# tier4/lidar_feature_extraction

Measured on AMD Instinct MI355X. Metric: scans/sec (64-ring x 1800 synthetic scans, extraction hot path, inputs resident in HBM), higher is better.
Workload: dtype f64

## Files before the change

### lidar_feature_extraction_amd/csrc/lfx_api.hip

```cpp
#include "lfx_internal.hpp"

#include <algorithm>
#include <cstddef>
#include "lfx_kernels_extract.hpp"

#ifdef LFX_TEST_HOOKS
#define LFX_DEBUG_ENV(name) std::getenv("LFX_DEBUG_" name)
#else
#define LFX_DEBUG_ENV(name) static_cast<const char *>(nullptr)
#endif

using namespace lfx_host;

namespace
{

std::string g_create_error;

const char * kKernelNames[LFX_N_KERNELS] = {
  "ring_scatter_kernel", "ring_unit_kernel", "ring_order_kernel", "ring_unit_kernel(second pass)", "ring_extract_kernel",
  "ring_totals_kernel", "feature_compact_kernel", "ring_unit_org_kernel", "ring_cut_kernel", "fallback_tail_kernel", "grid_count_kernel",
  "batch_reset_kernel", "ring_long_kernel",
  "pose_graph_linearize_kernel", "pose_graph_node_kernel", "pose_graph_reduce_kernel", "pose_graph_chain_factor_kernel",
  "pose_graph_chain_solve_kernel", "pose_graph_s_assemble_kernel", "pose_graph_s_diag_kernel", "pose_graph_s_panel_kernel",
  "pose_graph_s_update_kernel", "pose_graph_s_solve_kernel", "pose_graph_step_kernel"};

int64_t ordered_key(double d)
{
  int64_t k;
  std::memcpy(&k, &d, 8);
  return k < 0 ? std::numeric_limits<int64_t>::min() - k : k;
}

double from_ordered_key(int64_t k)
{
  const int64_t b = k < 0 ? std::numeric_limits<int64_t>::min() - k : k;
  double d;
  std::memcpy(&d, &b, 8);
  return d;
}

double cos_bound(double radian_threshold)
{
  if (!(std::acos(1.0) < radian_threshold)) {return std::numeric_limits<double>::infinity();}
  if (std::acos(-1.0) < radian_threshold) {return -1.0;}
  int64_t lo = ordered_key(-1.0), hi = ordered_key(1.0);
  while (hi - lo > 1) {
    const int64_t mid = lo + (hi - lo) / 2;
    if (std::acos(from_ordered_key(mid)) < radian_threshold) {hi = mid;} else {lo = mid;}
  }
  return from_ordered_key(hi);
}

}

std::string & lfx_host::create_error() {return g_create_error;}

namespace
{

struct Timed : TimedSpan
{
  Timed(lfx_ctx * c, KernelSlot k, hipStream_t s)
  : TimedSpan(c, c->profile_now, k, s) {}
};

int drain_spans(lfx_ctx * c)
{
  for (auto & sp : c->spans) {
    LFX_HIP(c, hipEventSynchronize(sp.b));
    float t = 0.f;
    LFX_HIP(c, hipEventElapsedTime(&t, sp.a, sp.b));
    c->ms[sp.k] += t;
    c->launches[sp.k] += 1;
    c->free_events.push_back(sp.a);
    c->free_events.push_back(sp.b);
  }
  c->spans.clear();
  return LFX_OK;
}

int validate_params(const lfx_params * p, std::string & why)
{
  if (!p) {why = "params is NULL"; return LFX_ERR_INVALID_ARGUMENT;}
  if (p->padding <= 0 || p->padding > LFX_MAX_PADDING) {
    why = "convolution_padding must be in [1, " + std::to_string(LFX_MAX_PADDING) + "]";
    return LFX_ERR_INVALID_ARGUMENT;
  }
  if (p->n_blocks <= 0) {why = "n_blocks must be > 0"; return LFX_ERR_INVALID_ARGUMENT;}
  if (!(p->neighbor_degree_threshold > 0) || !(p->distance_diff_threshold > 0) ||
    !(p->parallel_beam_min_range_ratio > 0) || !(p->edge_threshold > 0) || !(p->surface_threshold > 0) ||
    !(p->min_range > 0) || !(p->max_range > 0))
  {
    why = "every threshold / range parameter must be > 0 (hyper_parameter.hpp:45-53)";
    return LFX_ERR_INVALID_ARGUMENT;
  }
  return LFX_OK;
}

lfx::Params device_params(const lfx_params & p)
{
  lfx::Params d;
  d.P = p.padding;
  d.B = p.n_blocks;
  d.cos_bound = cos_bound(p.neighbor_degree_threshold * M_PI / 180.0);
  d.cos_bound_f = (float)d.cos_bound;
  d.dist_diff = p.distance_diff_threshold;
  d.pb_ratio = p.parallel_beam_min_range_ratio;
  d.pb_ratio_f = (float)d.pb_ratio;
  d.edge_thr = p.edge_threshold;
  d.surf_thr = p.surface_threshold;
  d.min_range = p.min_range;
  d.max_range = p.max_range;
  return d;
}

int debug_pin(const char * value) {return value ? (std::atoi(value) != 0 ? 1 : 0) : -1;}

// ... 131 lines not shown
      const uint32_t R = c->max_rings;
      const int P = c->dev.P, B = c->dev.B;
      for (uint32_t s = 0; s < batch; s++) {
        const uint32_t n = n_points[s], C = n / R;
        if (C * R != n || C == 0u || C > c->cap) {continue;}
        uint32_t * g = c->h_scan_geom.data() + (size_t)s * lfx::kGeomStride;
        g[0] = C;
        for (int j = 0; j <= B && j <= lfx::kUnitMaxBlocks; j++) {g[1 + j] = (uint32_t)lfx::block_boundary((int)C, P, B, j);}
      }
      LFX_HIP(c, hipMemcpyAsync(c->scan_geom.p, c->h_scan_geom.data(), c->h_scan_geom.size() * 4, hipMemcpyHostToDevice, st));
    }
  }
  c->last_batch = batch;
  c->last_points = d_points;
  c->deskewed_in_place = false;
  c->profile_now = c->profiling && (c->batch_no++ % c->profile_every) == 0u;
  const uint32_t par = c->parity;
  const AccSet acc = acc_set(c, par), other = acc_set(c, par ^ 1u);
  uint32_t * const counters = acc.counters;
  const lfx::UnitTables * unit_tab = c->unit_tab.p + par;
  uint32_t * defer_count = counters + lfx::kCntDefer, * redo_count = counters + lfx::kCntRedo,
    * slow_count = counters + lfx::kCntSlow, * fb_count = counters + lfx::kCntFallback;
  const uint8_t * pts = static_cast<const uint8_t *>(d_points);
  const uint32_t chunks = (longest + lfx::kChunkPoints - 1) / lfx::kChunkPoints;
  const bool canon = canonical_layout(c->layout) && (reinterpret_cast<uintptr_t>(pts) & 15u) == 0;
  if (c->long_slices != 0u) {
    LFX_HIP(c, hipMemsetAsync(c->long_count.p, 0, 4, st));
  }
  if (c->h_counters) {
    const uint32_t end = __atomic_load_n(c->h_counters + 1 + lfx::kCounters, __ATOMIC_ACQUIRE);
    uint32_t got[lfx::kCounters];
    for (int i = 0; i < lfx::kCounters; i++) {got[i] = __atomic_load_n(c->h_counters + 1 + i, __ATOMIC_RELAXED);}
    __atomic_thread_fence(__ATOMIC_ACQUIRE);
    const uint32_t begin = __atomic_load_n(c->h_counters, __ATOMIC_RELAXED);
    if (end != 0u && end == begin && end != c->report_taken) {
      static_assert(sizeof(c->route.report) == sizeof(got), "the report is the counters block");
      std::memcpy(c->route.report, got, sizeof(got));
      c->route.report_rings = got[lfx::kCntBatch] * c->max_rings;
      c->report_taken = end;
    }
  }
  const RouteChoice choice = choose_route(c->route, c->route_pins, c->fused_possible && canon && chunks != 0, batch, c->max_rings);
  const bool fused = choice.fused, short_tail = choice.short_tail;
  const bool holes = choice.holes && c->drop_zero != 0u && c->cum16.p != nullptr;
  const uint32_t fb_grid = choice.fb_grid;
  if (chunks == 0) {
    LFX_HIP(c, hipMemsetAsync(c->scan_info.p, 0, (size_t)batch * 16, st));
    LFX_HIP(c, hipMemsetAsync(c->ring_count.p, 0, (size_t)batch * lfx::kRings * 4, st));
    return LFX_OK;
  }
  const bool lazy = fused && short_tail && !choice.xform;
  if (!lazy || c->aux_dirty != 0u) {
    const uint32_t n_aux = c->aux_dirty > batch ? c->aux_dirty : batch;
    Timed t(c, kSlotReset, st);
    hipLaunchKernelGGL(lfx::batch_reset_kernel, dim3(64), dim3(256), 0, st,
      c->chunk_flags.p, n_aux * c->max_chunks, c->ring_flags.p, n_aux * (uint32_t)lfx::kRings, counters, c->fb_list.p, batch,
      fused ? 0u : 1u, c->xform.p);
    c->aux_dirty = lazy ? 0u : batch;
  }
  c->last_used_xform = fused && choice.xform;
  if (fused) {
    const bool xf = choice.xform;
    if (xf) {
      Timed t(c, kSlotCut, st);
      hipLaunchKernelGGL(lfx::ring_cut_kernel, dim3(batch), dim3(lfx::kCutThreads), 0, st,
        pts, c->scan_begin.p, c->max_rings, c->cap, c->xform.p, counters);
    }
    const uint32_t groups = (c->max_rings + 3u) / 4u;
    if (holes) {
      Timed t(c, kSlotGridCount, st);
      const uint32_t row_words = c->cap / lfx::kPieceCols + 1u;
      const size_t count_lds = ((size_t)c->max_rings * row_words + 2u * groups * (size_t)c->dev.B) * 4u;
      auto count_pass = [&](auto kernel, dim3 grid, uint32_t threads, size_t lds, auto... more) {
          hipLaunchKernelGGL(kernel, grid, dim3(threads), lds, st,
            pts, c->scan_begin.p, c->scan_geom.p, c->max_rings, lfx::cum_stride(c->cap), c->cum16.p, c->ring_count.p, unit_tab, counters,
            c->hole_desc.p, c->cap, 64u * c->unit_chunks, 4u * (uint32_t)lfx::holes_loads((int)c->unit_chunks), more...);
        };
      if (batch >= c->scan_count_from && count_lds <= 144u * 1024u) {
        count_pass(lfx::scan_count_kernel, dim3(batch), lfx::kScanCountThreads, count_lds, row_words);
      } else {
        count_pass(lfx::grid_count_kernel, dim3(groups, batch), 256u, 0);
      }
    }
    {
      Timed t(c, kSlotUnitOrg, st);
      const UnitOrgArgs a{c->dev, c->cap, c->unit_flags, c->max_rings, c->drop_zero, pts, c->scan_begin.p, c->ring_count.p, unit_tab,
        c->xform.p, c->scan_geom.p};
      launch_unit_org(c->unit_variant, (int)c->unit_chunks, xf, holes, dim3(groups, (uint32_t)c->dev.B, batch), c->unit_lds_pad, st, a);
    }
  }
  const lfx::RingExtractArgs ex{c->dev, c->cap, c->stage_flags, c->max_rings, pts, c->layout, c->scan_begin.p, c->ring_count.p, c->sxy.p, c->sz.p,
    c->sidx.p, c->label_s.p, (c->outputs & LFX_OUT_CURVATURE) ? c->curv_s.p : nullptr, c->rec_pts.p, c->rec_idx.p, c->ring_status.p,
    c->unit_ne.p, c->unit_ns.p, c->unit_span.p, c->ring_flags.p, c->long_count.p, c->long_list.p,
    (uint32_t)(c->long_list.n / 2u)};
  const lfx::ScatterArgs sc{pts, c->layout, c->scan_begin.p, c->chunk_base.p, c->chunk_flags.p, c->ring_count.p, c->scan_info.p, acc.scan_flags,
    c->sxy.p, c->sz.p, c->sidx.p, c->max_chunks, c->max_rings, c->cap, c->drop_zero};
  if (lazy) {
    Timed t(c, kSlotTail, st);
    const uint32_t turns = (batch + lfx::kTailMaxTurns - 1u) / lfx::kTailMaxTurns;
    const uint32_t rows = fb_grid < 2u ? fb_grid : 2u;
    const dim3 grid(chunks, rows > turns ? rows : turns);
    if (canon) {
      hipLaunchKernelGGL(lfx::fallback_tail_kernel<true>, grid, dim3(lfx::kChunkThreads), c->ring_lds, st, sc, ex, fb_count, c->fb_list.p, c->tail_ticket.p);
    } else {
      hipLaunchKernelGGL(lfx::fallback_tail_kernel<false>, grid, dim3(lfx::kChunkThreads), c->ring_lds, st, sc, ex, fb_count, c->fb_list.p, c->tail_ticket.p);
    }
  } else {
    {
      Timed t(c, kSlotScatter, st);
      auto kern = &lfx::ring_scatter_kernel<false>;
      if (canon) {kern = &lfx::ring_scatter_kernel<true>;}
      if (fb_grid == batch) {
        kern = canon ? &lfx::ring_scatter_kernel<true, true> : &lfx::ring_scatter_kernel<false, true>;
      }
      hipLaunchKernelGGL(kern, dim3(chunks, fb_grid), dim3(lfx::kChunkThreads), 0, st,
        sc.pts, sc.L, sc.scan_begin, sc.chunk_base, sc.chunk_flags, sc.ring_count, sc.scan_info, sc.scan_flags,
        sc.sxy, sc.sz, sc.sidx, sc.max_chunks, sc.max_rings, sc.cap, sc.drop_zero, fb_count, c->fb_list.p,
        c->slot_id.empty() ? nullptr : c->ring_slot.p);
    }
    const uint32_t list_grid = fused ? (c->slow_grid < 4u * fb_grid ? c->slow_grid : 4u * fb_grid) : c->slow_grid;
    if (c->fast_path && !short_tail) {
      auto order_pass = [&](uint32_t grid, uint32_t all_rings, uint32_t redo_cap, uint32_t list_cover) {
          Timed t(c, kSlotOrder, st);
          hipLaunchKernelGGL(lfx::ring_order_kernel, dim3(grid), dim3(512), c->order_lds, st,
            c->cap, c->max_rings, c->ring_count.p, c->sxy.p, c->sz.p, c->sidx.p, c->ring_flags.p, defer_count,
            c->defer_list.p, redo_count, c->redo_list.p, slow_count, c->slow_list.p, all_rings, counters + lfx::kCntPreFixed, redo_cap,
            fb_count, c->fb_list.p, list_cover);
        };
      c->pre_order = choice.pre_order;
      if (c->pre_order) {order_pass(fused ? list_grid : 4 * c->slow_grid, 1u, 0u, 0u);}
      {
        Timed t(c, kSlotUnit, st);
        const uint32_t units = c->max_rings * (uint32_t)c->dev.B;
        const UnitArgs a{c->dev, c->cap, c->unit_flags, c->max_rings, c->ring_count.p, c->sxy.p, c->sz.p, c->sidx.p, unit_tab,
          defer_count, c->defer_list.p, fb_count, c->fb_list.p, 0u};
        launch_unit(c->unit_variant, false, (int)c->unit_chunks, fused, dim3((units + lfx::kUnitWaves - 1) / lfx::kUnitWaves, fb_grid),
          c->unit_lds_pad, st, a);
      }
      const uint32_t redo_cap = choice.redo_cap;
      order_pass(list_grid, 0u, redo_cap, 0xFFFFFFFFu );
      {
        Timed t(c, kSlotUnitSecond, st);
        const uint32_t units = redo_cap * (uint32_t)c->dev.B;
        const UnitArgs a{c->dev, c->cap, c->unit_flags, c->max_rings, c->ring_count.p, c->sxy.p, c->sz.p, c->sidx.p, unit_tab,
          slow_count, c->slow_list.p, redo_count, c->redo_list.p, redo_cap};
        launch_unit(c->unit_variant, true, (int)c->unit_chunks, false, dim3((units + lfx::kUnitWaves - 1) / lfx::kUnitWaves), c->unit_lds_pad, st, a);
      }
    }
    {
      Timed t(c, kSlotExtract, st);
      const dim3 grid = c->fast_path ? dim3(list_grid) : dim3(c->max_rings, batch);
      hipLaunchKernelGGL(lfx::ring_extract_kernel, grid, dim3(c->ring_threads), c->ring_lds, st,
        ex, short_tail ? 2u : (c->fast_path ? 1u : 0u), short_tail ? fb_count : slow_count, short_tail ? c->fb_list.p : c->slow_list.p);
    }
  }
  if (c->long_slices != 0u) {
    Timed t(c, kSlotLong, st);
    hipLaunchKernelGGL(lfx::ring_long_kernel, dim3(c->long_slices), dim3(512), lfx::kLongSortLds, st, ex, c->long_work.p,
      c->long_slice_bytes);
  }
  {
    const uint32_t n_units = c->fast_path ? (uint32_t)c->dev.B : 1u;
    const bool self_totals = (fused || (uint64_t)batch * c->max_rings <= 8192u) && c->totals_env != 1;
    if (!self_totals) {
      Timed t(c, kSlotTotals, st);
      hipLaunchKernelGGL(lfx::ring_totals_kernel, dim3(batch), dim3(lfx::kRings), 0, st,
        c->scan_info.p, c->ring_count.p, c->unit_ne.p, c->unit_ns.p, acc.ring_nedge, acc.ring_nsurf,
        c->ring_ebase.p, c->ring_sbase.p, n_units, c->max_rings);
    }
    c->batch_serial = c->batch_serial + 1u == 0u ? 1u : c->batch_serial + 1u;
    {
      Timed t(c, kSlotCompact, st);
      hipLaunchKernelGGL(lfx::feature_compact_kernel, dim3((c->max_rings + 3) / 4, batch), dim3(256), 0, st,
        n_units, c->cap, c->scan_begin.p, c->ring_count.p, self_totals ? nullptr : c->ring_ebase.p, c->ring_sbase.p, c->unit_ne.p,
        c->unit_ns.p, c->unit_span.p, c->rec_pts.p, c->rec_idx.p, c->edge_pts.p, c->edge_idx.p, c->surf_pts.p,
        c->surf_idx.p, c->max_rings, c->scan_info.p, counters, c->h_counters, c->batch_serial, acc.ring_nedge, acc.ring_nsurf, c->rec32.p,
        c->slot_places, acc.scan_flags, c->ring_count.p, batch, fused ? 1u : 0u,
        other.counters, other.scan_flags, other.ring_nedge, other.ring_nsurf, c->par_dirty[par ^ 1u]);
    }
    c->par_dirty[par ^ 1u] = 0u;
    c->par_dirty[par] = batch;
    c->parity = par ^ 1u;
  }
  LFX_HIP(c, hipGetLastError());
  return LFX_OK;
}

size_t align16(size_t v) {return (v + 15u) & ~(size_t)15u;}

struct FetchPlan
{
  uint32_t first = 0, count = 0, p0 = 0, mask = 0;
  size_t o_hdr = 0, o_ep = 0, o_sp = 0, o_cv = 0, o_ei = 0, o_si = 0, o_sx = 0, o_lb = 0;
  uint8_t * H = nullptr;
  std::vector<uint32_t> begin;
};

int fetch_queue(lfx_ctx * c, uint32_t first, uint32_t count, hipStream_t st, uint32_t mask, PinnedBuf & block, FetchPlan & plan)
{
  if (count == 0 || first + count > c->last_batch) {return fail(c, LFX_ERR_INVALID_ARGUMENT, "scan index outside the last batch");}
  const uint32_t p0 = c->h_scan_begin[first];
  const size_t P = c->h_scan_begin[first + count] - p0;
  mask &= c->outputs | ~(uint32_t)LFX_OUT_CURVATURE;
  const bool want_lab = mask & LFX_OUT_LABELS, want_curv = mask & LFX_OUT_CURVATURE, want_sidx = mask & LFX_OUT_SORTED_INDEX;
  const size_t o_hdr = 0, o_ep = align16((size_t)count * lfx::kResultHeaderBytes), o_sp = o_ep + P * 16, o_cv = o_sp + P * 16,
    o_ei = o_cv + (want_curv ? P * 8 : 0), o_si = o_ei + P * 4, o_sx = o_si + P * 4, o_lb = o_sx + (want_sidx ? P * 4 : 0),
    total = o_lb + (want_lab ? P : 0) + 16;
  if (block.reserve(total) != hipSuccess) {return fail(c, LFX_ERR_OUT_OF_MEMORY, "cannot allocate the pinned result block");}
  uint8_t * H = block.p;
  plan.first = first; plan.count = count; plan.p0 = p0; plan.mask = mask; plan.H = H;
  plan.o_hdr = o_hdr; plan.o_ep = o_ep; plan.o_sp = o_sp; plan.o_cv = o_cv; plan.o_ei = o_ei; plan.o_si = o_si; plan.o_sx = o_sx; plan.o_lb = o_lb;
  plan.begin.assign(c->h_scan_begin.begin() + first, c->h_scan_begin.begin() + first + count + 1);
  hipLaunchKernelGGL(lfx::result_pack_kernel, dim3(8, count), dim3(256), 0, st,
    first, p0, c->scan_begin.p, c->scan_info.p, c->ring_count.p, c->ring_status.p, c->edge_pts.p, c->edge_idx.p,
    c->surf_pts.p, c->surf_idx.p, H + o_hdr, reinterpret_cast<float4 *>(H + o_ep), reinterpret_cast<float4 *>(H + o_sp),
    reinterpret_cast<uint32_t *>(H + o_ei), reinterpret_cast<uint32_t *>(H + o_si));
  LFX_HIP(c, hipGetLastError());
  if ((want_lab || want_curv || want_sidx) && P) {
    if (c->d_sidx.n < P) {
      LFX_HIP(c, hipStreamSynchronize(st));
      c->d_label.release(); c->d_curv.release(); c->d_sidx.release();
      if (c->d_label.alloc(P) != hipSuccess || c->d_curv.alloc(P) != hipSuccess || c->d_sidx.alloc(P) != hipSuccess) {
        return fail(c, LFX_ERR_OUT_OF_MEMORY, "cannot allocate the per-point output buffers");
      }
    }
    LFX_HIP(c, hipMemsetAsync(c->d_label.p, 0, P, st));
// ... 895 lines not shown
```

### lidar_feature_extraction_amd/csrc/lfx_internal.hpp

```cpp
#pragma once

#include "../../include/lfx.h"

#include <hip/hip_runtime.h>

#include <cmath>
#include <cstdio>
#include <cstdlib>
#include <cstring>
#include <limits>
#include <string>
#include <type_traits>
#include <utility>
#include <vector>

#include "lfx_kernels_common.hpp"

namespace lfx_host
{

constexpr int kUnitVariantPadding[4] = {5, 5, 2, 0};

struct UnitOrgArgs
{
  lfx::Params prm;
  uint32_t cap, flags, max_rings, drop_zero;
  const uint8_t * pts;
  const uint32_t * scan_begin;
  uint32_t * ring_count;
  const lfx::UnitTables * tab;
  const uint32_t * xform, * geom;
};
struct UnitArgs
{
  lfx::Params prm;
  uint32_t cap, flags, max_rings;
  const uint32_t * ring_count;
  const float2 * sxy;
  const float * sz;
  const uint32_t * sidx;
  const lfx::UnitTables * tab;
  uint32_t * defer_count, * defer_list;
  const uint32_t * list_count, * list;
  uint32_t redo_cap;
};
#define LFX_DECLARE_UNIT_LAUNCHERS(V) \
  void launch_unit_org_v##V(int chunks, bool xf, bool holes, dim3 grid, uint32_t lds_pad, hipStream_t st, const UnitOrgArgs & a); \
  void launch_unit_v##V(bool second, int chunks, bool loop, dim3 grid, uint32_t lds_pad, hipStream_t st, const UnitArgs & a);
LFX_DECLARE_UNIT_LAUNCHERS(0) LFX_DECLARE_UNIT_LAUNCHERS(1) LFX_DECLARE_UNIT_LAUNCHERS(2) LFX_DECLARE_UNIT_LAUNCHERS(3)
#undef LFX_DECLARE_UNIT_LAUNCHERS
inline void launch_unit_org(int variant, int chunks, bool xf, bool holes, dim3 grid, uint32_t lds_pad, hipStream_t st, const UnitOrgArgs & a)
{
  switch (variant) {
    case 0: launch_unit_org_v0(chunks, xf, holes, grid, lds_pad, st, a); break;
    case 1: launch_unit_org_v1(chunks, xf, holes, grid, lds_pad, st, a); break;
    case 2: launch_unit_org_v2(chunks, xf, holes, grid, lds_pad, st, a); break;
    default: launch_unit_org_v3(chunks, xf, holes, grid, lds_pad, st, a); break;
  }
}
inline void launch_unit(int variant, bool second, int chunks, bool loop, dim3 grid, uint32_t lds_pad, hipStream_t st, const UnitArgs & a)
{
  switch (variant) {
    case 0: launch_unit_v0(second, chunks, loop, grid, lds_pad, st, a); break;
    case 1: launch_unit_v1(second, chunks, loop, grid, lds_pad, st, a); break;
    case 2: launch_unit_v2(second, chunks, loop, grid, lds_pad, st, a); break;
    default: launch_unit_v3(second, chunks, loop, grid, lds_pad, st, a); break;
  }
}

template<typename T>
struct DevBuf
{
  T * p = nullptr;
  size_t n = 0;
  DevBuf() = default;
  DevBuf(const DevBuf &) = delete;
  DevBuf & operator=(const DevBuf &) = delete;
  DevBuf(DevBuf && o) noexcept : p(o.p), n(o.n) {o.p = nullptr; o.n = 0;}
  DevBuf & operator=(DevBuf && o) noexcept
  {
    if (this != &o) {release(); p = o.p; n = o.n; o.p = nullptr; o.n = 0;}
    return *this;
  }
  ~DevBuf() {release();}
  hipError_t alloc(size_t count)
  {
    release();
    const hipError_t e = hipMalloc(reinterpret_cast<void **>(&p), count * sizeof(T) + 16);
    if (e == hipSuccess) {n = count;} else {p = nullptr;}
    return e;
  }
  void release()
  {
    if (p) {(void)hipFree(p);}
    p = nullptr;
    n = 0;
  }
};
static_assert(!std::is_copy_constructible_v<DevBuf<float>> && !std::is_copy_assignable_v<DevBuf<float>>, "a device buffer has one owner");

template<typename T>
hipError_t hold(DevBuf<T> & b, size_t need, bool exact = false)
{
  if (b.n >= need && (b.p || need == 0)) {return hipSuccess;}
  return b.alloc(exact ? need : need + need / 2);
}

struct HostScan
{
  std::vector<uint8_t> ring_status;
  std::vector<uint32_t> ring_count, ring_offset;
  std::vector<uint16_t> ring_id;
};

struct PinnedBuf
{
  uint8_t * p = nullptr;
  size_t bytes = 0;
  PinnedBuf() = default;
// ... 212 lines not shown

  bool profiling = false;
  uint32_t profile_every = 1, batch_no = 0;
  bool profile_now = false;
  struct Span { hipEvent_t a, b; int k; };
  std::vector<Span> spans;
  std::vector<hipEvent_t> free_events;
  double ms[LFX_N_KERNELS] = {};
  uint64_t launches[LFX_N_KERNELS] = {};
};

namespace lfx_host
{

std::string & create_error();

inline hipEvent_t take_event(lfx_ctx * c)
{
  if (!c->free_events.empty()) {
    hipEvent_t e = c->free_events.back();
    c->free_events.pop_back();
    return e;
  }
  hipEvent_t e = nullptr;
  (void)hipEventCreate(&e);
  return e;
}
struct TimedSpan
{
  TimedSpan(lfx_ctx * c, bool on, int k, hipStream_t s)
  : c_(c), on_(on), k_(k), s_(s)
  {
    if (on_) {
      a_ = take_event(c_);
      b_ = take_event(c_);
      (void)hipEventRecord(a_, s_);
    }
  }
  ~TimedSpan()
  {
    if (on_) {
      (void)hipEventRecord(b_, s_);
      c_->spans.push_back({a_, b_, k_});
    }
  }
  TimedSpan(const TimedSpan &) = delete;
  TimedSpan & operator=(const TimedSpan &) = delete;
  lfx_ctx * c_;
  bool on_;
  int k_;
  hipStream_t s_;
  hipEvent_t a_ = nullptr, b_ = nullptr;
};

#define LFX_HIP(ctx, call) \
  do { \
    const hipError_t e_ = (call); \
    if (e_ != hipSuccess) { \
      (ctx)->err = std::string(#call) + ": " + hipGetErrorString(e_); \
      return LFX_ERR_HIP; \
    } \
  } while (0)

inline int fail(lfx_ctx * ctx, int code, const std::string & msg)
{
  if (ctx) {ctx->err = msg;}
  return code;
}

inline int Tail::order_behind(lfx_ctx * c, hipStream_t st) const
{
  if (pending) {LFX_HIP(c, hipStreamWaitEvent(st, event, 0));}
  return LFX_OK;
}
inline int Tail::done(lfx_ctx * c, hipStream_t st) const
{
  if (!event) {LFX_HIP(c, hipEventCreateWithFlags(&event, hipEventDisableTiming));}
  LFX_HIP(c, hipEventRecord(event, st));
  pending = true;
  return LFX_OK;
}
inline int Tail::settle(lfx_ctx * c) const
{
  if (pending) {LFX_HIP(c, hipEventSynchronize(event)); pending = false;}
  return LFX_OK;
}

inline int TableSlot::take(lfx_ctx * c, size_t doubles, hipError_t & mem)
{
  const int rs = used.settle(c);
  if (rs != LFX_OK) {return rs;}
  mem = h.reserve(sizeof(double) * doubles);
  if (mem == hipSuccess) {mem = hold(d, doubles);}
  return LFX_OK;
}

inline int check_device(lfx_ctx * c, int device, const char * what)
{
  if (device != c->device) {return fail(c, LFX_ERR_INVALID_ARGUMENT, std::string(what) + " lives on another device");}
  return LFX_OK;
}

inline bool finite_all(const double * v, size_t n)
{
  for (size_t i = 0; i < n; i++) {
    if (!std::isfinite(v[i])) {return false;}
// ... 123 lines not shown
```

### lidar_feature_extraction_amd/csrc/lfx_kernels_extract.hpp

```cpp
#pragma once

#include "lfx_kernels_common.hpp"

#pragma clang fp contract(off)

namespace lfx
{

__global__ __launch_bounds__(256) void batch_reset_kernel(
  uint32_t * __restrict__ chunk_flags, uint32_t n_flags, uint32_t * __restrict__ ring_flags, uint32_t n_rflags,
  uint32_t * __restrict__ counters , uint32_t * __restrict__ fb_list, uint32_t batch,
  uint32_t all_fall_back ,
  uint32_t * __restrict__ xform )
{
  const uint32_t i = blockIdx.x * blockDim.x + threadIdx.x, stride = gridDim.x * blockDim.x;
  for (uint32_t k = i; k < n_flags; k += stride) {chunk_flags[k] = 0;}
  for (uint32_t k = i; k < n_rflags; k += stride) {ring_flags[k] = 0; xform[k] = 0;}
  if (all_fall_back) {
    for (uint32_t k = i; k < batch; k += stride) {fb_list[k] = k;}
    if (i == 0) {counters[kCntFallback] = batch;}
  }
}

constexpr uint32_t kSpinLimit = 200000;
// ... 1993 lines not shown
    if (n_scan == 0u) {
      if (lane == 0) {
        ring_count_w[s * kRings + slot] = 0u;
        if (slot == 0u) {
          scan_info[s * 4 + kInfoRings] = 0u; scan_info[s * 4 + kInfoError] = err_pub;
          scan_info[s * 4 + kInfoEdge] = 0u; scan_info[s * 4 + kInfoSurface] = 0u;
        }
      }
      return;
    }
    if (slot == 0u && lane == 0) {scan_info[s * 4 + kInfoError] = err_pub;}
    if (slot == max_rings - 1u && (err & (kScanHoles | kScanFellBack)) == kScanHoles) {
      uint32_t occupied = 0;
      for (uint32_t r = lane; r < max_rings; r += 64) {occupied += ring_count[s * kRings + r] != 0u ? 1u : 0u;}
      occupied = (uint32_t)__builtin_amdgcn_readlane((int)wave_inclusive_sum(occupied), 63);
      if (lane == 0) {scan_info[s * 4 + kInfoRings] = occupied;}
    }
    const bool by_ring = scan_is_organised(err);
    size_t eb, fb;
    if (ring_ebase) {
      eb = b + e_base;
      fb = b + f_base;
    } else {
      uint32_t e = e_before, f = f_before;
      if (!by_ring) {
        e = 0; f = 0;
        for (uint32_t r = lane; r < slot; r += 64) {
          if (ring_count[s * kRings + r] != 0u) {
            const size_t ur = ((size_t)s * kRings + r) * kUnitMaxBlocks;
            for (uint32_t j = 0; j < n_units; j++) {e += unit_ne[ur + j]; f += unit_ns[ur + j];}
          }
        }
      }
      e = (uint32_t)__builtin_amdgcn_readlane((int)wave_inclusive_sum(e), 63);
      f = (uint32_t)__builtin_amdgcn_readlane((int)wave_inclusive_sum(f), 63);
      eb = b + e;
      fb = b + f;
      if (slot == max_rings - 1u) {
        uint32_t oe = n_ring != 0u ? ne_k : 0u, of = n_ring != 0u ? ns_k : 0u;
        oe = (uint32_t)__builtin_amdgcn_readlane((int)wave_inclusive_sum(oe), 63);
        of = (uint32_t)__builtin_amdgcn_readlane((int)wave_inclusive_sum(of), 63);
        if (lane == 0) {
          scan_info[s * 4 + kInfoEdge] = e + oe;
          scan_info[s * 4 + kInfoSurface] = f + of;
        }
      }
    }
    if (n_ring == 0u) {return;}
    const size_t off = ring_base(s, slot, max_rings, cap);
    const uint32_t tot_k = ne_k + ns_k;
    const uint32_t incl = wave_inclusive_sum(tot_k), e_incl = wave_inclusive_sum(ne_k), s_incl = wave_inclusive_sum(ns_k);
    const uint32_t total = (uint32_t)__builtin_amdgcn_readlane((int)incl, 63);
    const uint32_t excl = incl - tot_k, e_excl = e_incl - ne_k, s_excl = s_incl - ns_k;
    for (uint32_t t0 = 0; t0 < total; t0 += 256) {
      size_t src[4], dst[4];
      uint32_t idx_at[4];
      bool edge[4], valid[4], in_slot[4];
#pragma unroll
      for (int i = 0; i < 4; i++) {
        const uint32_t t = t0 + 64 * i + lane;
        valid[i] = t < total;
        uint32_t u = 0;
        for (uint32_t v = 0; v + 1u < n_units; v++) {u += t >= (uint32_t)__builtin_amdgcn_readlane((int)incl, (int)v) ? 1u : 0u;}
        const uint32_t ne = (uint32_t)__shfl((int)ne_k, (int)u), ns = (uint32_t)__shfl((int)ns_k, (int)u), span = (uint32_t)__shfl((int)span_k, (int)u);
        const uint32_t cum = (uint32_t)__shfl((int)excl, (int)u), ecum = (uint32_t)__shfl((int)e_excl, (int)u), scum = (uint32_t)__shfl((int)s_excl, (int)u);
        const size_t first = off + (span & 0xFFFFu), last = off + ((span & kUnitWholeRing) != 0u ? n_ring : ((span >> 16) & 0x7FFFu));
        const bool slots = (span & kUnitRecordsInSlot) != 0u;
        const uint32_t q = t - cum;
        edge[i] = q < ne;
        in_slot[i] = slots && q < slot_places;
        idx_at[i] = 4u * (ne + ns < slot_places ? ne + ns : slot_places) - 3u * q;
        if (slots) {
          src[i] = in_slot[i] ? (((size_t)s * max_rings + slot) * n_units + u) * (slot_places * (kRecBytes / 4u)) + 4u * q : first + q;
        } else {
          src[i] = edge[i] ? first + q : last - 1 - (q - ne);
        }
        dst[i] = edge[i] ? eb + ecum + q : fb + scum + (q - ne);
        if (!valid[i]) {src[i] = off; dst[i] = b; in_slot[i] = false;}
      }
      float4 rp[4];
      uint32_t ri[4];
#pragma unroll
      for (int i = 0; i < 4; i++) {
        rp[i] = make_float4(0.f, 0.f, 0.f, 0.f);
        ri[i] = 0;
        if (valid[i]) {
          if (in_slot[i]) {
            const uint32_t * w = reinterpret_cast<const uint32_t *>(rec32) + src[i];
            rp[i] = *reinterpret_cast<const float4 *>(w);
            ri[i] = w[idx_at[i]];
          } else {
            rp[i] = rec_pts[src[i]];
            ri[i] = rec_idx[src[i]];
          }
        }
      }
#pragma unroll
      for (int i = 0; i < 4; i++) {
        if (valid[i]) {
          if (edge[i]) {
            edge_pts[dst[i]] = rp[i];
            edge_idx[dst[i]] = ri[i];
          } else {
            surf_pts[dst[i]] = rp[i];
            surf_idx[dst[i]] = ri[i];
          }
        }
      }
    }
  }
}

__global__ __launch_bounds__(256) void densify_kernel(
  uint32_t first, uint32_t p0, const uint32_t * __restrict__ scan_begin, uint32_t max_rings, uint32_t cap,
  const uint32_t * __restrict__ ring_count,
  const uint8_t * __restrict__ label_s, const double * __restrict__ curv_s, const uint32_t * __restrict__ sidx,
  uint8_t * __restrict__ d_label, double * __restrict__ d_curv, uint32_t * __restrict__ d_sidx,
  const uint32_t * __restrict__ scan_info, const uint32_t * __restrict__ xform)
{
  const uint32_t s = first + blockIdx.y;
  const uint32_t at = scan_begin[s] - p0, n_points = scan_begin[s + 1] - scan_begin[s];
  d_label += at; d_curv += at; d_sidx += at;
  const uint32_t ring = blockIdx.x, tid = threadIdx.x;
  const bool org = scan_is_grid(scan_info[s * 4 + kInfoError]);
  __shared__ uint32_t part[256];
  part[tid] = (tid < ring && tid < max_rings) ? ring_count[s * kRings + tid] : 0u;
  __syncthreads();
  for (int d = 128; d > 0; d >>= 1) {
    if ((int)tid < d) {part[tid] += part[tid + d];}
    __syncthreads();
  }
  const uint32_t dense = part[0];
  uint32_t N = ring_count[s * kRings + ring];
  N = N < cap ? N : cap;
  const size_t off = ring_base(s, ring, max_rings, cap);
  const uint32_t Nfull = ring_count[s * kRings + ring];
  for (uint32_t i = tid; i < Nfull; i += blockDim.x) {
    const bool stored = i < N;
    const uint32_t orig = stored ? (org ? ring_column(xform[s * kRings + ring], i, Nfull) * max_rings + ring : sidx[off + i]) : 0xFFFFFFFFu;
    d_sidx[dense + i] = orig;
    if (orig < n_points) {
      d_label[orig] = label_s[off + i];
      if (curv_s != nullptr) {d_curv[orig] = curv_s[off + i];}
    }
  }
}

constexpr uint32_t kResultHeaderBytes = 16 + kRings * 4 + kRings;
__global__ __launch_bounds__(256) void result_pack_kernel(
  uint32_t first, uint32_t p0, const uint32_t * __restrict__ scan_begin, const uint32_t * __restrict__ scan_info,
  const uint32_t * __restrict__ ring_count, const uint8_t * __restrict__ ring_status,
  const float4 * __restrict__ edge_pts, const uint32_t * __restrict__ edge_idx, const float4 * __restrict__ surf_pts,
  const uint32_t * __restrict__ surf_idx, uint8_t * __restrict__ h_hdr, float4 * __restrict__ h_edge_pts,
  float4 * __restrict__ h_surf_pts, uint32_t * __restrict__ h_edge_idx, uint32_t * __restrict__ h_surf_idx)
{
  const uint32_t k = blockIdx.y, s = first + k, tid = threadIdx.x;
  if (blockIdx.x == 0) {
    uint32_t * hdr = reinterpret_cast<uint32_t *>(h_hdr + (size_t)k * kResultHeaderBytes);
// ... 63 lines not shown
```

Measured before the change: 922,400.

## Record profiling events inside kernel launches and use 32-bit addressing in compaction

Replaces the RAII timing spans that wrapped each launch with hipExtLaunchKernelGGL, which records the start and stop events as part of the launch itself when profiling is on. When profiling is off, launches go through plain hipLaunchKernelGGL. Separately, the feature compaction loop now builds per-ring base pointers in the global address space once and indexes them with 32-bit byte offsets, instead of computing 64-bit element indices for each load and store. This is meant to cut address arithmetic and register pressure in the compact kernel, and to cut host-side event calls when profiling. The 32-bit offsets assume each per-ring region stays under 4 GiB.

```diff
diff --git a/lidar_feature_extraction_amd/csrc/lfx_api.hip b/lidar_feature_extraction_amd/csrc/lfx_api.hip
--- a/lidar_feature_extraction_amd/csrc/lfx_api.hip
+++ b/lidar_feature_extraction_amd/csrc/lfx_api.hip
@@ -59,11 +59,7 @@
 namespace
 {
 
-struct Timed : TimedSpan
-{
-  Timed(lfx_ctx * c, KernelSlot k, hipStream_t s)
-  : TimedSpan(c, c->profile_now, k, s) {}
-};
+LaunchSpan timed(lfx_ctx * c, KernelSlot k) {return launch_span(c, c->profile_now, k);}
 
 int drain_spans(lfx_ctx * c)
 {
@@ -301,8 +297,7 @@
   const bool lazy = fused && short_tail && !choice.xform;
   if (!lazy || c->aux_dirty != 0u) {
     const uint32_t n_aux = c->aux_dirty > batch ? c->aux_dirty : batch;
-    Timed t(c, kSlotReset, st);
-    hipLaunchKernelGGL(lfx::batch_reset_kernel, dim3(64), dim3(256), 0, st,
+    launch_kernel(timed(c, kSlotReset), lfx::batch_reset_kernel, dim3(64), dim3(256), 0, st,
       c->chunk_flags.p, n_aux * c->max_chunks, c->ring_flags.p, n_aux * (uint32_t)lfx::kRings, counters, c->fb_list.p, batch,
       fused ? 0u : 1u, c->xform.p);
     c->aux_dirty = lazy ? 0u : batch;
@@ -311,17 +306,15 @@
   if (fused) {
     const bool xf = choice.xform;
     if (xf) {
-      Timed t(c, kSlotCut, st);
-      hipLaunchKernelGGL(lfx::ring_cut_kernel, dim3(batch), dim3(lfx::kCutThreads), 0, st,
+      launch_kernel(timed(c, kSlotCut), lfx::ring_cut_kernel, dim3(batch), dim3(lfx::kCutThreads), 0, st,
         pts, c->scan_begin.p, c->max_rings, c->cap, c->xform.p, counters);
     }
     const uint32_t groups = (c->max_rings + 3u) / 4u;
     if (holes) {
-      Timed t(c, kSlotGridCount, st);
       const uint32_t row_words = c->cap / lfx::kPieceCols + 1u;
       const size_t count_lds = ((size_t)c->max_rings * row_words + 2u * groups * (size_t)c->dev.B) * 4u;
       auto count_pass = [&](auto kernel, dim3 grid, uint32_t threads, size_t lds, auto... more) {
-          hipLaunchKernelGGL(kernel, grid, dim3(threads), lds, st,
+          launch_kernel(timed(c, kSlotGridCount), kernel, grid, dim3(threads), lds, st,
             pts, c->scan_begin.p, c->scan_geom.p, c->max_rings, lfx::cum_stride(c->cap), c->cum16.p, c->ring_count.p, unit_tab, counters,
             c->hole_desc.p, c->cap, 64u * c->unit_chunks, 4u * (uint32_t)lfx::holes_loads((int)c->unit_chunks), more...);
         };
@@ -332,10 +325,10 @@
       }
     }
     {
-      Timed t(c, kSlotUnitOrg, st);
       const UnitOrgArgs a{c->dev, c->cap, c->unit_flags, c->max_rings, c->drop_zero, pts, c->scan_begin.p, c->ring_count.p, unit_tab,
         c->xform.p, c->scan_geom.p};
-      launch_unit_org(c->unit_variant, (int)c->unit_chunks, xf, holes, dim3(groups, (uint32_t)c->dev.B, batch), c->unit_lds_pad, st, a);
+      launch_unit_org(c->unit_variant, (int)c->unit_chunks, xf, holes, dim3(groups, (uint32_t)c->dev.B, batch), c->unit_lds_pad, st, a,
+        timed(c, kSlotUnitOrg));
     }
   }
   const lfx::RingExtractArgs ex{c->dev, c->cap, c->stage_flags, c->max_rings, pts, c->layout, c->scan_begin.p, c->ring_count.p, c->sxy.p, c->sz.p,
@@ -345,24 +338,22 @@
   const lfx::ScatterArgs sc{pts, c->layout, c->scan_begin.p, c->chunk_base.p, c->chunk_flags.p, c->ring_count.p, c->scan_info.p, acc.scan_flags,
     c->sxy.p, c->sz.p, c->sidx.p, c->max_chunks, c->max_rings, c->cap, c->drop_zero};
   if (lazy) {
-    Timed t(c, kSlotTail, st);
     const uint32_t turns = (batch + lfx::kTailMaxTurns - 1u) / lfx::kTailMaxTurns;
     const uint32_t rows = fb_grid < 2u ? fb_grid : 2u;
     const dim3 grid(chunks, rows > turns ? rows : turns);
     if (canon) {
-      hipLaunchKernelGGL(lfx::fallback_tail_kernel<true>, grid, dim3(lfx::kChunkThreads), c->ring_lds, st, sc, ex, fb_count, c->fb_list.p, c->tail_ticket.p);
+      launch_kernel(timed(c, kSlotTail), lfx::fallback_tail_kernel<true>, grid, dim3(lfx::kChunkThreads), c->ring_lds, st, sc, ex, fb_count, c->fb_list.p, c->tail_ticket.p);
     } else {
-      hipLaunchKernelGGL(lfx::fallback_tail_kernel<false>, grid, dim3(lfx::kChunkThreads), c->ring_lds, st, sc, ex, fb_count, c->fb_list.p, c->tail_ticket.p);
+      launch_kernel(timed(c, kSlotTail), lfx::fallback_tail_kernel<false>, grid, dim3(lfx::kChunkThreads), c->ring_lds, st, sc, ex, fb_count, c->fb_list.p, c->tail_ticket.p);
     }
   } else {
     {
-      Timed t(c, kSlotScatter, st);
       auto kern = &lfx::ring_scatter_kernel<false>;
       if (canon) {kern = &lfx::ring_scatter_kernel<true>;}
       if (fb_grid == batch) {
         kern = canon ? &lfx::ring_scatter_kernel<true, true> : &lfx::ring_scatter_kernel<false, true>;
       }
-      hipLaunchKernelGGL(kern, dim3(chunks, fb_grid), dim3(lfx::kChunkThreads), 0, st,
+      launch_kernel(timed(c, kSlotScatter), kern, dim3(chunks, fb_grid), dim3(lfx::kChunkThreads), 0, st,
         sc.pts, sc.L, sc.scan_begin, sc.chunk_base, sc.chunk_flags, sc.ring_count, sc.scan_info, sc.scan_flags,
         sc.sxy, sc.sz, sc.sidx, sc.max_chunks, sc.max_rings, sc.cap, sc.drop_zero, fb_count, c->fb_list.p,
         c->slot_id.empty() ? nullptr : c->ring_slot.p);
@@ -370,8 +361,7 @@
     const uint32_t list_grid = fused ? (c->slow_grid < 4u * fb_grid ? c->slow_grid : 4u * fb_grid) : c->slow_grid;
     if (c->fast_path && !short_tail) {
       auto order_pass = [&](uint32_t grid, uint32_t all_rings, uint32_t redo_cap, uint32_t list_cover) {
-          Timed t(c, kSlotOrder, st);
-          hipLaunchKernelGGL(lfx::ring_order_kernel, dim3(grid), dim3(512), c->order_lds, st,
+          launch_kernel(timed(c, kSlotOrder), lfx::ring_order_kernel, dim3(grid), dim3(512), c->order_lds, st,
             c->cap, c->max_rings, c->ring_count.p, c->sxy.p, c->sz.p, c->sidx.p, c->ring_flags.p, defer_count,
             c->defer_list.p, redo_count, c->redo_list.p, slow_count, c->slow_list.p, all_rings, counters + lfx::kCntPreFixed, redo_cap,
             fb_count, c->fb_list.p, list_cover);
@@ -379,48 +369,43 @@
       c->pre_order = choice.pre_order;
       if (c->pre_order) {order_pass(fused ? list_grid : 4 * c->slow_grid, 1u, 0u, 0u);}
       {
-        Timed t(c, kSlotUnit, st);
         const uint32_t units = c->max_rings * (uint32_t)c->dev.B;
         const UnitArgs a{c->dev, c->cap, c->unit_flags, c->max_rings, c->ring_count.p, c->sxy.p, c->sz.p, c->sidx.p, unit_tab,
           defer_count, c->defer_list.p, fb_count, c->fb_list.p, 0u};
         launch_unit(c->unit_variant, false, (int)c->unit_chunks, fused, dim3((units + lfx::kUnitWaves - 1) / lfx::kUnitWaves, fb_grid),
-          c->unit_lds_pad, st, a);
+          c->unit_lds_pad, st, a, timed(c, kSlotUnit));
       }
       const uint32_t redo_cap = choice.redo_cap;
       order_pass(list_grid, 0u, redo_cap, 0xFFFFFFFFu );
       {
-        Timed t(c, kSlotUnitSecond, st);
         const uint32_t units = redo_cap * (uint32_t)c->dev.B;
         const UnitArgs a{c->dev, c->cap, c->unit_flags, c->max_rings, c->ring_count.p, c->sxy.p, c->sz.p, c->sidx.p, unit_tab,
           slow_count, c->slow_list.p, redo_count, c->redo_list.p, redo_cap};
-        launch_unit(c->unit_variant, true, (int)c->unit_chunks, false, dim3((units + lfx::kUnitWaves - 1) / lfx::kUnitWaves), c->unit_lds_pad, st, a);
+        launch_unit(c->unit_variant, true, (int)c->unit_chunks, false, dim3((units + lfx::kUnitWaves - 1) / lfx::kUnitWaves), c->unit_lds_pad, st, a,
+          timed(c, kSlotUnitSecond));
       }
     }
     {
-      Timed t(c, kSlotExtract, st);
       const dim3 grid = c->fast_path ? dim3(list_grid) : dim3(c->max_rings, batch);
-      hipLaunchKernelGGL(lfx::ring_extract_kernel, grid, dim3(c->ring_threads), c->ring_lds, st,
+      launch_kernel(timed(c, kSlotExtract), lfx::ring_extract_kernel, grid, dim3(c->ring_threads), c->ring_lds, st,
         ex, short_tail ? 2u : (c->fast_path ? 1u : 0u), short_tail ? fb_count : slow_count, short_tail ? c->fb_list.p : c->slow_list.p);
     }
   }
   if (c->long_slices != 0u) {
-    Timed t(c, kSlotLong, st);
-    hipLaunchKernelGGL(lfx::ring_long_kernel, dim3(c->long_slices), dim3(512), lfx::kLongSortLds, st, ex, c->long_work.p,
+    launch_kernel(timed(c, kSlotLong), lfx::ring_long_kernel, dim3(c->long_slices), dim3(512), lfx::kLongSortLds, st, ex, c->long_work.p,
       c->long_slice_bytes);
   }
   {
     const uint32_t n_units = c->fast_path ? (uint32_t)c->dev.B : 1u;
     const bool self_totals = (fused || (uint64_t)batch * c->max_rings <= 8192u) && c->totals_env != 1;
     if (!self_totals) {
-      Timed t(c, kSlotTotals, st);
-      hipLaunchKernelGGL(lfx::ring_totals_kernel, dim3(batch), dim3(lfx::kRings), 0, st,
+      launch_kernel(timed(c, kSlotTotals), lfx::ring_totals_kernel, dim3(batch), dim3(lfx::kRings), 0, st,
         c->scan_info.p, c->ring_count.p, c->unit_ne.p, c->unit_ns.p, acc.ring_nedge, acc.ring_nsurf,
         c->ring_ebase.p, c->ring_sbase.p, n_units, c->max_rings);
     }
     c->batch_serial = c->batch_serial + 1u == 0u ? 1u : c->batch_serial + 1u;
     {
-      Timed t(c, kSlotCompact, st);
-      hipLaunchKernelGGL(lfx::feature_compact_kernel, dim3((c->max_rings + 3) / 4, batch), dim3(256), 0, st,
+      launch_kernel(timed(c, kSlotCompact), lfx::feature_compact_kernel, dim3((c->max_rings + 3) / 4, batch), dim3(256), 0, st,
         n_units, c->cap, c->scan_begin.p, c->ring_count.p, self_totals ? nullptr : c->ring_ebase.p, c->ring_sbase.p, c->unit_ne.p,
         c->unit_ns.p, c->unit_span.p, c->rec_pts.p, c->rec_idx.p, c->edge_pts.p, c->edge_idx.p, c->surf_pts.p,
         c->surf_idx.p, c->max_rings, c->scan_info.p, counters, c->h_counters, c->batch_serial, acc.ring_nedge, acc.ring_nsurf, c->rec32.p,
diff --git a/lidar_feature_extraction_amd/csrc/lfx_internal.hpp b/lidar_feature_extraction_amd/csrc/lfx_internal.hpp
--- a/lidar_feature_extraction_amd/csrc/lfx_internal.hpp
+++ b/lidar_feature_extraction_amd/csrc/lfx_internal.hpp
@@ -3,6 +3,7 @@
 #include "../../include/lfx.h"
 
 #include <hip/hip_runtime.h>
+#include <hip/hip_ext.h>
 
 #include <cmath>
 #include <cstdio>
@@ -20,6 +21,20 @@
 {
 
 constexpr int kUnitVariantPadding[4] = {5, 5, 2, 0};
+
+struct LaunchSpan
+{
+  hipEvent_t a = nullptr, b = nullptr;
+};
+template<typename ... P, typename ... A>
+inline void launch_kernel(const LaunchSpan & sp, void (* kernel)(P...), dim3 grid, dim3 block, size_t lds, hipStream_t st, A && ... args)
+{
+  if (sp.a != nullptr) {
+    hipExtLaunchKernelGGL(kernel, grid, block, (uint32_t)lds, st, sp.a, sp.b, 0u, static_cast<P>(args)...);
+  } else {
+    hipLaunchKernelGGL(kernel, grid, block, lds, st, static_cast<P>(args)...);
+  }
+}
 
 struct UnitOrgArgs
 {
@@ -45,26 +60,26 @@
   uint32_t redo_cap;
 };
 #define LFX_DECLARE_UNIT_LAUNCHERS(V) \
-  void launch_unit_org_v##V(int chunks, bool xf, bool holes, dim3 grid, uint32_t lds_pad, hipStream_t st, const UnitOrgArgs & a); \
-  void launch_unit_v##V(bool second, int chunks, bool loop, dim3 grid, uint32_t lds_pad, hipStream_t st, const UnitArgs & a);
+  void launch_unit_org_v##V(int chunks, bool xf, bool holes, dim3 grid, uint32_t lds_pad, hipStream_t st, const UnitOrgArgs & a, const LaunchSpan & sp); \
+  void launch_unit_v##V(bool second, int chunks, bool loop, dim3 grid, uint32_t lds_pad, hipStream_t st, const UnitArgs & a, const LaunchSpan & sp);
 LFX_DECLARE_UNIT_LAUNCHERS(0) LFX_DECLARE_UNIT_LAUNCHERS(1) LFX_DECLARE_UNIT_LAUNCHERS(2) LFX_DECLARE_UNIT_LAUNCHERS(3)
 #undef LFX_DECLARE_UNIT_LAUNCHERS
-inline void launch_unit_org(int variant, int chunks, bool xf, bool holes, dim3 grid, uint32_t lds_pad, hipStream_t st, const UnitOrgArgs & a)
+inline void launch_unit_org(int variant, int chunks, bool xf, bool holes, dim3 grid, uint32_t lds_pad, hipStream_t st, const UnitOrgArgs & a, const LaunchSpan & sp)
 {
   switch (variant) {
-    case 0: launch_unit_org_v0(chunks, xf, holes, grid, lds_pad, st, a); break;
-    case 1: launch_unit_org_v1(chunks, xf, holes, grid, lds_pad, st, a); break;
-    case 2: launch_unit_org_v2(chunks, xf, holes, grid, lds_pad, st, a); break;
-    default: launch_unit_org_v3(chunks, xf, holes, grid, lds_pad, st, a); break;
-  }
-}
-inline void launch_unit(int variant, bool second, int chunks, bool loop, dim3 grid, uint32_t lds_pad, hipStream_t st, const UnitArgs & a)
+    case 0: launch_unit_org_v0(chunks, xf, holes, grid, lds_pad, st, a, sp); break;
+    case 1: launch_unit_org_v1(chunks, xf, holes, grid, lds_pad, st, a, sp); break;
+    case 2: launch_unit_org_v2(chunks, xf, holes, grid, lds_pad, st, a, sp); break;
+    default: launch_unit_org_v3(chunks, xf, holes, grid, lds_pad, st, a, sp); break;
+  }
+}
+inline void launch_unit(int variant, bool second, int chunks, bool loop, dim3 grid, uint32_t lds_pad, hipStream_t st, const UnitArgs & a, const LaunchSpan & sp)
 {
   switch (variant) {
-    case 0: launch_unit_v0(second, chunks, loop, grid, lds_pad, st, a); break;
-    case 1: launch_unit_v1(second, chunks, loop, grid, lds_pad, st, a); break;
-    case 2: launch_unit_v2(second, chunks, loop, grid, lds_pad, st, a); break;
-    default: launch_unit_v3(second, chunks, loop, grid, lds_pad, st, a); break;
+    case 0: launch_unit_v0(second, chunks, loop, grid, lds_pad, st, a, sp); break;
+    case 1: launch_unit_v1(second, chunks, loop, grid, lds_pad, st, a, sp); break;
+    case 2: launch_unit_v2(second, chunks, loop, grid, lds_pad, st, a, sp); break;
+    default: launch_unit_v3(second, chunks, loop, grid, lds_pad, st, a, sp); break;
   }
 }
 
@@ -383,6 +398,16 @@
   hipStream_t s_;
   hipEvent_t a_ = nullptr, b_ = nullptr;
 };
+inline LaunchSpan launch_span(lfx_ctx * c, bool on, int k)
+{
+  LaunchSpan sp;
+  if (on) {
+    sp.a = take_event(c);
+    sp.b = take_event(c);
+    c->spans.push_back({sp.a, sp.b, k});
+  }
+  return sp;
+}
 
 #define LFX_HIP(ctx, call) \
   do { \
diff --git a/lidar_feature_extraction_amd/csrc/lfx_kernels_extract.hpp b/lidar_feature_extraction_amd/csrc/lfx_kernels_extract.hpp
--- a/lidar_feature_extraction_amd/csrc/lfx_kernels_extract.hpp
+++ b/lidar_feature_extraction_amd/csrc/lfx_kernels_extract.hpp
@@ -2069,10 +2069,23 @@
     const uint32_t incl = wave_inclusive_sum(tot_k), e_incl = wave_inclusive_sum(ne_k), s_incl = wave_inclusive_sum(ns_k);
     const uint32_t total = (uint32_t)__builtin_amdgcn_readlane((int)incl, 63);
     const uint32_t excl = incl - tot_k, e_excl = e_incl - ne_k, s_excl = s_incl - ns_k;
+    typedef __attribute__((address_space(1))) const uint8_t g_cu8_t;
+    typedef __attribute__((address_space(1))) uint8_t g_u8_t;
+    typedef __attribute__((address_space(1))) const uint32_t g_cu32_t;
+    typedef __attribute__((address_space(1))) uint32_t g_u32_t;
+    typedef float f32x4_t __attribute__((ext_vector_type(4)));
+    typedef __attribute__((address_space(1))) const f32x4_t g_cf32x4_t;
+    typedef __attribute__((address_space(1))) f32x4_t g_f32x4_t;
+    const uint32_t slot_bytes = slot_places * kRecBytes;
+    g_cu8_t * const slots_u = (g_cu8_t *)rec32 + (((size_t)s * max_rings + slot) * n_units) * slot_bytes;
+    g_cu8_t * const pts_u = (g_cu8_t *)(rec_pts + off), * const idx_u = (g_cu8_t *)(rec_idx + off);
+    g_u8_t * const epts_u = (g_u8_t *)(edge_pts + eb), * const eidx_u = (g_u8_t *)(edge_idx + eb);
+    g_u8_t * const spts_u = (g_u8_t *)(surf_pts + fb), * const sidx_u = (g_u8_t *)(surf_idx + fb);
     for (uint32_t t0 = 0; t0 < total; t0 += 256) {
-      size_t src[4], dst[4];
-      uint32_t idx_at[4];
-      bool edge[4], valid[4], in_slot[4];
+      uint32_t dst[4];
+      bool edge[4], valid[4];
+      f32x4_t rp[4];
+      uint32_t ri[4];
 #pragma unroll
       for (int i = 0; i < 4; i++) {
         const uint32_t t = t0 + 64 * i + lane;
@@ -2081,34 +2094,23 @@
         for (uint32_t v = 0; v + 1u < n_units; v++) {u += t >= (uint32_t)__builtin_amdgcn_readlane((int)incl, (int)v) ? 1u : 0u;}
         const uint32_t ne = (uint32_t)__shfl((int)ne_k, (int)u), ns = (uint32_t)__shfl((int)ns_k, (int)u), span = (uint32_t)__shfl((int)span_k, (int)u);
         const uint32_t cum = (uint32_t)__shfl((int)excl, (int)u), ecum = (uint32_t)__shfl((int)e_excl, (int)u), scum = (uint32_t)__shfl((int)s_excl, (int)u);
-        const size_t first = off + (span & 0xFFFFu), last = off + ((span & kUnitWholeRing) != 0u ? n_ring : ((span >> 16) & 0x7FFFu));
+        const uint32_t first = span & 0xFFFFu, last = (span & kUnitWholeRing) != 0u ? n_ring : ((span >> 16) & 0x7FFFu);
         const bool slots = (span & kUnitRecordsInSlot) != 0u;
         const uint32_t q = t - cum;
         edge[i] = q < ne;
-        in_slot[i] = slots && q < slot_places;
-        idx_at[i] = 4u * (ne + ns < slot_places ? ne + ns : slot_places) - 3u * q;
-        if (slots) {
-          src[i] = in_slot[i] ? (((size_t)s * max_rings + slot) * n_units + u) * (slot_places * (kRecBytes / 4u)) + 4u * q : first + q;
-        } else {
-          src[i] = edge[i] ? first + q : last - 1 - (q - ne);
-        }
-        dst[i] = edge[i] ? eb + ecum + q : fb + scum + (q - ne);
-        if (!valid[i]) {src[i] = off; dst[i] = b; in_slot[i] = false;}
-      }
-      float4 rp[4];
-      uint32_t ri[4];
-#pragma unroll
-      for (int i = 0; i < 4; i++) {
-        rp[i] = make_float4(0.f, 0.f, 0.f, 0.f);
+        dst[i] = edge[i] ? ecum + q : scum + (q - ne);
+        rp[i] = f32x4_t{0.f, 0.f, 0.f, 0.f};
         ri[i] = 0;
         if (valid[i]) {
-          if (in_slot[i]) {
-            const uint32_t * w = reinterpret_cast<const uint32_t *>(rec32) + src[i];
-            rp[i] = *reinterpret_cast<const float4 *>(w);
-            ri[i] = w[idx_at[i]];
+          if (slots && q < slot_places) {
+            const uint32_t n_in = ne + ns < slot_places ? ne + ns : slot_places;
+            const uint32_t at = u * slot_bytes + 16u * q;
+            rp[i] = *(g_cf32x4_t *)(slots_u + at);
+            ri[i] = *(g_cu32_t *)(slots_u + (at + 4u * (4u * n_in - 3u * q)));
           } else {
-            rp[i] = rec_pts[src[i]];
-            ri[i] = rec_idx[src[i]];
+            const uint32_t r = slots || edge[i] ? first + q : last - 1u - (q - ne);
+            rp[i] = *(g_cf32x4_t *)(pts_u + 16u * r);
+            ri[i] = *(g_cu32_t *)(idx_u + 4u * r);
           }
         }
       }
@@ -2116,11 +2118,11 @@
       for (int i = 0; i < 4; i++) {
         if (valid[i]) {
           if (edge[i]) {
-            edge_pts[dst[i]] = rp[i];
-            edge_idx[dst[i]] = ri[i];
+            *(g_f32x4_t *)(epts_u + 16u * dst[i]) = rp[i];
+            *(g_u32_t *)(eidx_u + 4u * dst[i]) = ri[i];
           } else {
-            surf_pts[dst[i]] = rp[i];
-            surf_idx[dst[i]] = ri[i];
+            *(g_f32x4_t *)(spts_u + 16u * dst[i]) = rp[i];
+            *(g_u32_t *)(sidx_u + 4u * dst[i]) = ri[i];
           }
         }
       }
```

Result: no change. 927,200 (median of 5 runs) (+0.5%).
